# earth-insights/ZoomEarth

Measured on NVIDIA B200. Metric: vision tokens/s crop->patchify->ViT, higher is better.
Workload: dtype fp16

## Files before the change

include/zoomvit.h:

```cpp
#ifndef ZOOMVIT_H_
#define ZOOMVIT_H_

#include <stddef.h>
#include <stdint.h>

#ifdef __cplusplus
extern "C" {
#endif

#define ZV_API __attribute__((visibility("default")))

typedef enum zv_err {
  ZV_OK = 0,
  ZV_EINVAL = -1,
  ZV_EINVAL_ASPECT = -2,
  ZV_EINVAL_BOX = -3,
  ZV_ENOMEM = -4,
  ZV_ECUDA = -5,
  ZV_ENODEV = -6,
  ZV_EARCH = -7
} zv_err;

enum { ZV_F32 = 0, ZV_BF16 = 1, ZV_F16 = 2 };
enum { ZV_ORDER_HF = 0, ZV_ORDER_WINDOW = 1 };
enum { ZV_TOWER_QWEN25 = 0, ZV_TOWER_QWEN2 = 1 };

typedef struct zv_cfg {
  int32_t patch;
  int32_t merge;
  int32_t temporal;
  int32_t window;
  int32_t min_size;
  int32_t depth;
  int32_t hidden;
  int32_t heads;
  int32_t inter;
  int32_t out_hidden;
  int32_t fullatt_mask_lo;
  int32_t op_dtype;
  int64_t min_pixels;
  int64_t max_pixels;
  double  rescale;
  float   mean[3];
  float   std[3];
  float   eps;
  float   reserved_f;
  int32_t tower_kind;
  int32_t reserved_i;
} zv_cfg;

ZV_API const char* zv_version(void);
ZV_API const char* zv_last_error(void);
ZV_API void zv_default_cfg(zv_cfg* cfg);

ZV_API int zv_cut_box(int32_t img_w, int32_t img_h, const double* bbox_xyxy, int32_t min_size, int32_t* box_out4);
ZV_API int zv_resize_dims(int32_t w, int32_t h, int32_t max_size, int32_t* new_wh2, double* inv_scale);
ZV_API int zv_resize_dims_ex(int32_t w, int32_t h, int32_t max_size, int32_t mode, int32_t* new_wh2, double* inv_scale);
ZV_API int zv_cut_box_sft(int32_t img_w, int32_t img_h, const double* bbox_xyxy, int32_t min_size, int32_t* box_out4,
                          int32_t* resized_wh2, int32_t* centre_box4);
ZV_API int zv_smart_resize(int32_t height, int32_t width, int32_t factor, int64_t min_pixels, int64_t max_pixels,
                           int32_t* out_hw2);
ZV_API int zv_geometry(const zv_cfg* cfg, int32_t n, const int32_t* img_hw, const double* bbox_xyxy,
                       int32_t* crop_box, int32_t* resized_hw, int64_t* grid_thw);

ZV_API int32_t zv_resample_ksize(int32_t in_size, int32_t out_size);
ZV_API int zv_resample_coeffs(int32_t in_size, int32_t out_size, int32_t* bounds, int32_t* kk);
ZV_API int zv_normalize_lut(const zv_cfg* cfg, float* lut768);

ZV_API int64_t zv_preprocess_workspace_bytes(int32_t n, const int32_t* crop_box, const int32_t* resized_hw);
ZV_API int zv_preprocess(const zv_cfg* cfg, int32_t n, const uint8_t* const* src_dev, const int32_t* src_hw,
                         const int64_t* src_pitch, const int32_t* crop_box, const int32_t* resized_hw,
                         const int64_t* row_off, void* out_dev, int32_t out_dtype, int32_t row_order,
                         void* workspace_dev, int64_t workspace_bytes, void* stream);

ZV_API int64_t zv_resize_u8_workspace_bytes(int32_t n, const int32_t* crop_box, const int32_t* out_hw);
ZV_API int zv_resize_u8(int32_t n, const uint8_t* const* src_dev, const int32_t* src_hw, const int64_t* src_pitch,
                        const int32_t* crop_box, const int32_t* out_hw, uint8_t* const* dst_dev, const int64_t* dst_pitch,
                        void* workspace_dev, int64_t workspace_bytes, void* stream);

ZV_API int zv_debug_k1_tc_host(const zv_cfg* cfg, int32_t n, const uint8_t* const* src_host, const int32_t* src_hw,
                               const int64_t* src_pitch, const int32_t* crop_box, const int32_t* resized_hw, float* out_host,
                               int32_t row_order, uint8_t* const* u8_dst_host, const int64_t* u8_pitch, void* workspace_host,
                               int64_t workspace_bytes, int32_t* took_tc);

typedef struct zv_plan zv_plan;
ZV_API int zv_plan_create(const zv_cfg* cfg, int32_t n, const int64_t* grid_thw, zv_plan** out);
ZV_API void zv_plan_free(zv_plan* p);
ZV_API int64_t zv_plan_num_patches(const zv_plan* p);
ZV_API int64_t zv_plan_num_tokens(const zv_plan* p);
ZV_API const int64_t* zv_plan_window_index(const zv_plan* p);
ZV_API const int64_t* zv_plan_reverse_index(const zv_plan* p);
ZV_API const int32_t* zv_plan_cu_window(const zv_plan* p, int32_t* n_out);
ZV_API const int32_t* zv_plan_cu_window_raw(const zv_plan* p, int32_t* n_out);
ZV_API const int32_t* zv_plan_cu_full(const zv_plan* p, int32_t* n_out);
ZV_API const int32_t* zv_plan_pos_ids(const zv_plan* p);
ZV_API int64_t zv_plan_device_bytes(const zv_plan* p);
ZV_API int zv_plan_upload(zv_plan* p, void* plan_dev, int64_t bytes, void* stream);

typedef struct zv_tensor {
  const char* name;
  const void* data;
  int32_t dtype;
  int32_t ndim;
  int64_t shape[5];
} zv_tensor;
ZV_API int64_t zv_weights_bytes(const zv_cfg* cfg);
ZV_API int zv_weights_pack(const zv_cfg* cfg, const zv_tensor* tensors, int32_t n, void* packed_dev,
                           int64_t packed_bytes, void* stream);

ZV_API int64_t zv_visual_workspace_bytes(const zv_cfg* cfg, const zv_plan* p);
ZV_API int zv_visual_forward(const zv_cfg* cfg, const void* weights_dev, const zv_plan* p, const void* plan_dev,
                             const void* patches_dev, int32_t in_dtype, int32_t in_order, void* merged_out_dev,
                             int32_t out_dtype, void* hidden_out_dev, void* workspace_dev,
                             int64_t workspace_bytes, void* stream);
ZV_API int zv_visual_forward_gather(const zv_cfg* cfg, const void* weights_dev, const zv_plan* p, const void* plan_dev,
                                    const void* patches_dev, int32_t in_dtype, int32_t in_order, void* merged_out_dev,
                                    int32_t out_dtype, void* workspace_dev, int64_t workspace_bytes,
                                    void* const* peer_out_dev, int32_t n_peers, int64_t peer_row_off, void* stream);
ZV_API int zv_visual_forward_gather_rows(const zv_cfg* cfg, const void* weights_dev, const zv_plan* p, const void* plan_dev,
                                         const void* patches_dev, int32_t in_dtype, int32_t in_order, void* gather_local_dev,
                                         int64_t gather_rows, int32_t out_dtype, const int64_t* dest_rows_dev,
                                         void* workspace_dev, int64_t workspace_bytes, void* const* peer_out_dev,
                                         int32_t n_peers, void* stream);
ZV_API int zv_visual_forward_into(const zv_cfg* cfg, const void* weights_dev, const zv_plan* p, const void* plan_dev,
                                  const void* patches_dev, int32_t in_dtype, int32_t in_order, void* embeds_dev,
                                  int64_t embeds_rows, int32_t embeds_dtype, const int64_t* dest_rows_dev,
                                  void* workspace_dev, int64_t workspace_bytes, void* stream);

ZV_API int zv_rope_index(const int64_t* input_ids, const int64_t* attention_mask, int32_t batch, int32_t seq_len,
                         const int64_t* image_grid_thw, int32_t n_images, int64_t image_token_id,
                         int64_t video_token_id, int64_t vision_start_token_id, int32_t merge, int32_t hf5_semantics,
                         int64_t* position_ids, int64_t* deltas);
ZV_API int64_t zv_placeholder_rows(const int64_t* input_ids, int64_t n_tokens, int64_t image_token_id,
                                   int64_t* rows_out, int64_t rows_cap);

ZV_API int64_t zv_last_launch_count(void);

ZV_API void zv_timing_enable(int on);
ZV_API void zv_timing_reset(void);
ZV_API int zv_timing_read(int kernel_class, double* ms_total, int64_t* count);

ZV_API int zv_gemm_bf16(const void* a_dev, int64_t lda, const void* b_dev, int64_t ldb, const float* bias_dev,
                        void* c_dev, int64_t ldc, int32_t c_dtype, int64_t m, int64_t n, int64_t k,
                        void* stream);
ZV_API int zv_gemm_ex(int32_t epilogue, const void* a_dev, int64_t lda, const void* b_dev, int64_t ldb,
                      const float* bias_dev, void* out_dev, int64_t ldo, int32_t out_dtype, int64_t m, int64_t n,
                      int64_t k, const int32_t* pos_dev, const float* rope_dev, const int32_t* scatter_dev,
                      int32_t heads, int32_t op_dtype , void* stream);
ZV_API int zv_attention(const void* qkv_dev, void* out_dev, int32_t heads, int32_t head_dim,
                        const int32_t* cu_seqlens_host, int32_t n_seg, void* work_dev, int64_t work_bytes,
                        int32_t dtype , void* stream);

#ifdef __cplusplus
}
#endif
#endif
```

zoomearth_b200/_lib.py:

```python
import ctypes as C
import os

_HERE = os.path.dirname(os.path.abspath(__file__))
LIB_PATH = os.path.join(_HERE, "libzoomvit.so")

ZV_F32, ZV_BF16, ZV_F16 = 0, 1, 2
ORDER_HF, ORDER_WINDOW = 0, 1
TOWER_QWEN25, TOWER_QWEN2 = 0, 1
ZV_EINVAL, ZV_EINVAL_ASPECT, ZV_EINVAL_BOX, ZV_ENOMEM, ZV_ECUDA, ZV_ENODEV, ZV_EARCH = -1, -2, -3, -4, -5, -6, -7


class ZvCfg(C.Structure):
    _fields_ = [
        ("patch", C.c_int32), ("merge", C.c_int32), ("temporal", C.c_int32), ("window", C.c_int32),
        ("min_size", C.c_int32), ("depth", C.c_int32), ("hidden", C.c_int32), ("heads", C.c_int32),
        ("inter", C.c_int32), ("out_hidden", C.c_int32), ("fullatt_mask_lo", C.c_int32), ("op_dtype", C.c_int32),
        ("min_pixels", C.c_int64), ("max_pixels", C.c_int64), ("rescale", C.c_double),
        ("mean", C.c_float * 3), ("std", C.c_float * 3), ("eps", C.c_float), ("reserved_f", C.c_float),
        ("tower_kind", C.c_int32), ("reserved_i", C.c_int32),
    ]


class ZvTensor(C.Structure):
    _fields_ = [("name", C.c_char_p), ("data", C.c_void_p), ("dtype", C.c_int32), ("ndim", C.c_int32),
                ("shape", C.c_int64 * 5)]


class ZoomVitError(RuntimeError):
    def __init__(self, code, msg):
        super().__init__(f"libzoomvit error {code}: {msg}")
        self.code = code
        self.msg = msg


_P = C.POINTER
_PROTOS = {
    "zv_version": (C.c_char_p, []),
    "zv_last_error": (C.c_char_p, []),
    "zv_default_cfg": (None, [_P(ZvCfg)]),
    "zv_cut_box": (C.c_int, [C.c_int32, C.c_int32, _P(C.c_double), C.c_int32, _P(C.c_int32)]),
    "zv_resize_dims": (C.c_int, [C.c_int32, C.c_int32, C.c_int32, _P(C.c_int32), _P(C.c_double)]),
    "zv_resize_dims_ex": (C.c_int, [C.c_int32, C.c_int32, C.c_int32, C.c_int32, _P(C.c_int32), _P(C.c_double)]),
    "zv_cut_box_sft": (C.c_int, [C.c_int32, C.c_int32, _P(C.c_double), C.c_int32, _P(C.c_int32), _P(C.c_int32), _P(C.c_int32)]),
    "zv_resize_u8_workspace_bytes": (C.c_int64, [C.c_int32, C.c_void_p, C.c_void_p]),
    "zv_resize_u8": (C.c_int, [C.c_int32, C.c_void_p, C.c_void_p, C.c_void_p, C.c_void_p, C.c_void_p, C.c_void_p, C.c_void_p,
                              C.c_void_p, C.c_int64, C.c_void_p]),
    "zv_smart_resize": (C.c_int, [C.c_int32, C.c_int32, C.c_int32, C.c_int64, C.c_int64, _P(C.c_int32)]),
    "zv_geometry": (C.c_int, [_P(ZvCfg), C.c_int32, C.c_void_p, C.c_void_p, C.c_void_p, C.c_void_p, C.c_void_p]),
    "zv_resample_ksize": (C.c_int32, [C.c_int32, C.c_int32]),
    "zv_resample_coeffs": (C.c_int, [C.c_int32, C.c_int32, C.c_void_p, C.c_void_p]),
    "zv_normalize_lut": (C.c_int, [_P(ZvCfg), C.c_void_p]),
    "zv_preprocess_workspace_bytes": (C.c_int64, [C.c_int32, C.c_void_p, C.c_void_p]),
    "zv_preprocess": (C.c_int, [_P(ZvCfg), C.c_int32, C.c_void_p, C.c_void_p, C.c_void_p, C.c_void_p, C.c_void_p,
                                C.c_void_p, C.c_void_p, C.c_int32, C.c_int32, C.c_void_p, C.c_int64, C.c_void_p]),
    "zv_debug_k1_tc_host": (C.c_int, [_P(ZvCfg), C.c_int32, C.c_void_p, C.c_void_p, C.c_void_p, C.c_void_p, C.c_void_p, C.c_void_p,
                                     C.c_int32, C.c_void_p, C.c_void_p, C.c_void_p, C.c_int64, C.c_void_p]),
    "zv_plan_create": (C.c_int, [_P(ZvCfg), C.c_int32, C.c_void_p, _P(C.c_void_p)]),
    "zv_plan_free": (None, [C.c_void_p]),
    "zv_plan_num_patches": (C.c_int64, [C.c_void_p]),
    "zv_plan_num_tokens": (C.c_int64, [C.c_void_p]),
    "zv_plan_window_index": (_P(C.c_int64), [C.c_void_p]),
    "zv_plan_reverse_index": (_P(C.c_int64), [C.c_void_p]),
    "zv_plan_cu_window": (_P(C.c_int32), [C.c_void_p, _P(C.c_int32)]),
    "zv_plan_cu_window_raw": (_P(C.c_int32), [C.c_void_p, _P(C.c_int32)]),
    "zv_plan_cu_full": (_P(C.c_int32), [C.c_void_p, _P(C.c_int32)]),
    "zv_plan_pos_ids": (_P(C.c_int32), [C.c_void_p]),
    "zv_plan_device_bytes": (C.c_int64, [C.c_void_p]),
    "zv_plan_upload": (C.c_int, [C.c_void_p, C.c_void_p, C.c_int64, C.c_void_p]),
    "zv_weights_bytes": (C.c_int64, [_P(ZvCfg)]),
    "zv_weights_pack": (C.c_int, [_P(ZvCfg), _P(ZvTensor), C.c_int32, C.c_void_p, C.c_int64, C.c_void_p]),
    "zv_visual_workspace_bytes": (C.c_int64, [_P(ZvCfg), C.c_void_p]),
    "zv_visual_forward": (C.c_int, [_P(ZvCfg), C.c_void_p, C.c_void_p, C.c_void_p, C.c_void_p, C.c_int32, C.c_int32,
                                    C.c_void_p, C.c_int32, C.c_void_p, C.c_void_p, C.c_int64, C.c_void_p]),
    "zv_visual_forward_gather": (C.c_int, [_P(ZvCfg), C.c_void_p, C.c_void_p, C.c_void_p, C.c_void_p, C.c_int32, C.c_int32,
                                           C.c_void_p, C.c_int32, C.c_void_p, C.c_int64, C.c_void_p, C.c_int32, C.c_int64,
                                           C.c_void_p]),
    "zv_visual_forward_gather_rows": (C.c_int, [_P(ZvCfg), C.c_void_p, C.c_void_p, C.c_void_p, C.c_void_p, C.c_int32, C.c_int32,
                                                C.c_void_p, C.c_int64, C.c_int32, C.c_void_p, C.c_void_p, C.c_int64, C.c_void_p,
                                                C.c_int32, C.c_void_p]),
    "zv_visual_forward_into": (C.c_int, [_P(ZvCfg), C.c_void_p, C.c_void_p, C.c_void_p, C.c_void_p, C.c_int32, C.c_int32,
                                         C.c_void_p, C.c_int64, C.c_int32, C.c_void_p, C.c_void_p, C.c_int64, C.c_void_p]),
    "zv_rope_index": (C.c_int, [C.c_void_p, C.c_void_p, C.c_int32, C.c_int32, C.c_void_p, C.c_int32, C.c_int64, C.c_int64,
                                C.c_int64, C.c_int32, C.c_int32, C.c_void_p, C.c_void_p]),
    "zv_placeholder_rows": (C.c_int64, [C.c_void_p, C.c_int64, C.c_int64, C.c_void_p, C.c_int64]),
    "zv_last_launch_count": (C.c_int64, []),
    "zv_timing_enable": (None, [C.c_int]),
    "zv_timing_reset": (None, []),
    "zv_timing_read": (C.c_int, [C.c_int, _P(C.c_double), _P(C.c_int64)]),
    "zv_gemm_bf16": (C.c_int, [C.c_void_p, C.c_int64, C.c_void_p, C.c_int64, C.c_void_p, C.c_void_p, C.c_int64,
                               C.c_int32, C.c_int64, C.c_int64, C.c_int64, C.c_void_p]),
    "zv_gemm_ex": (C.c_int, [C.c_int32, C.c_void_p, C.c_int64, C.c_void_p, C.c_int64, C.c_void_p, C.c_void_p, C.c_int64,
                             C.c_int32, C.c_int64, C.c_int64, C.c_int64, C.c_void_p, C.c_void_p, C.c_void_p, C.c_int32,
                             C.c_int32, C.c_void_p]),
    "zv_attention": (C.c_int, [C.c_void_p, C.c_void_p, C.c_int32, C.c_int32, C.c_void_p, C.c_int32, C.c_void_p,
                               C.c_int64, C.c_int32, C.c_void_p]),
}
EXPORTS = tuple(_PROTOS)
_lib = None


def lib():
    global _lib
    if _lib is None:
        if not os.path.exists(LIB_PATH):
            raise ImportError(
                f"{LIB_PATH} is missing: run `python -m zoomearth_b200.build` (nvcc, sm_100a). "
                "zoomearth_b200 has no CPU or PyTorch fallback path.")
        handle = C.CDLL(LIB_PATH)
        for name, (res, args) in _PROTOS.items():
            fn = getattr(handle, name)
            fn.restype = res
            fn.argtypes = args
        _lib = handle
    return _lib


def check(rc):
    if rc is not None and rc < 0:
        raise ZoomVitError(rc, lib().zv_last_error().decode())
    return rc


def default_cfg(**overrides):
    cfg = ZvCfg()
    lib().zv_default_cfg(C.byref(cfg))
    for k, v in overrides.items():
        if k in ("mean", "std"):
            setattr(cfg, k, (C.c_float * 3)(*v))
        elif k == "fullatt":
            m = 0
            for i in v:
                m |= 1 << i
            cfg.fullatt_mask_lo = m - (1 << 32) if m >= (1 << 31) else m
        else:
            setattr(cfg, k, v)
    return cfg
```

zoomearth_b200/csrc/zv_gemm.cu:

```cuda
#include <cuda.h>
#include <cuda_bf16.h>
#include <cuda_fp16.h>
#include <cuda_runtime.h>

#include <cstdlib>
#include <mutex>

#include "zv_common.h"
#include "zv_gemm.h"
#include "zv_ptx.cuh"

namespace zv {

using namespace ptx;

namespace {

constexpr int BM = 128, BK = 64, UMMA_K = 16;
constexpr int kThreads = 384;
constexpr int kTmemCols = 512;

constexpr int kXposePitch = 36;
constexpr int kXposeBytesPerWarp = 32 * kXposePitch * 4;
constexpr int kQkvRope0 = 24 * 32 * 8, kQkvRope1 = 16 * 32 * 8, kQkvTilePitch = 88, kQkvTile = 32 * kQkvTilePitch * 2;
constexpr int kQkvStageBytes = 4 * kQkvRope0 + 4 * kQkvRope1 + 4 * kQkvTile;
__host__ __device__ constexpr bool is_resid(int e) { return e == EPI_RESID || e == EPI_RESID_LN; }
__host__ __device__ constexpr bool is_qkv(int e) { return e == EPI_QKV_ROPE || e == EPI_QKV_ROPE_LN; }
template <int BN, int CG, int EPI = 0> struct Cfg {
  static constexpr int kBRows = BN / CG;
  static constexpr int kABytes = BM * BK * 2;
  static constexpr int kBBytes = kBRows * BK * 2;
  static constexpr int kStageBytes = kABytes + kBBytes;
  static constexpr int kXposeBytes = (is_resid(EPI) || EPI == EPI_SCATTER) ? 8 * kXposeBytesPerWarp : is_qkv(EPI) ? kQkvStageBytes : 0;
  static constexpr int kStages = ((kBRows > 128) ? 4 : 6) - ((is_resid(EPI) || is_qkv(EPI) || EPI == EPI_SCATTER) ? 1 : 0);
  static constexpr int kBarBytes = 256;
  static constexpr int kSmemBytes = kStages * kStageBytes + kBarBytes + kXposeBytes + 1024;
};

__device__ __forceinline__ float silu(float x) { return __fdividef(x, 1.0f + __expf(-x)); }
__device__ __forceinline__ float quick_gelu(float x) { return __fdividef(x, 1.0f + __expf(-1.702f * x)); }
__device__ __forceinline__ float gelu_erf(float x) { return 0.5f * x * (1.0f + erff(x * 0.70710678118654752440f)); }
__device__ __forceinline__ uint32_t pack2(float a, float b, bool f16) {
  if (f16) { __half2 v = __floats2half2_rn(a, b); return *reinterpret_cast<uint32_t*>(&v); }
  __nv_bfloat162 v = __floats2bfloat162_rn(a, b);
  return *reinterpret_cast<uint32_t*>(&v);
}
__device__ __forceinline__ void tmem_ld_x8(uint32_t taddr, uint32_t (&r)[8]) {
  asm volatile("tcgen05.ld.sync.aligned.32x32b.x8.b32 {%0, %1, %2, %3, %4, %5, %6, %7}, [%8];"
               : "=r"(r[0]), "=r"(r[1]), "=r"(r[2]), "=r"(r[3]), "=r"(r[4]), "=r"(r[5]), "=r"(r[6]), "=r"(r[7])
               : "r"(taddr) : "memory");
}
__device__ __forceinline__ void load_bias32(const float* __restrict__ b, float (&v)[32]) {
  const float4* p = reinterpret_cast<const float4*>(b);
#pragma unroll
  for (int j = 0; j < 8; ++j) { const float4 t = __ldg(p + j); v[4 * j] = t.x; v[4 * j + 1] = t.y; v[4 * j + 2] = t.z; v[4 * j + 3] = t.w; }
}

__device__ __forceinline__ float row_rscale(const GemmArgs& g, int row, bool valid) {
  if (g.row_ss == nullptr || !valid) return 1.f;
  const float2* p = reinterpret_cast<const float2*>(g.row_ss + (int64_t)row * kSsParts);
  float s = 0.f;
#pragma unroll
  for (int i = 0; i < kSsParts / 2; ++i) { const float2 t = __ldg(p + i); s += t.x; s += t.y; }
  return rsqrtf(s / (float)g.norm_dim + g.norm_eps);
}

__device__ __forceinline__ void row_ln_stats(const GemmArgs& g, int row, bool valid, float& mu, float& rs) {
  mu = 0.f; rs = 1.f;
  if (!valid) return;
  const float4* p = reinterpret_cast<const float4*>(g.row_ln + (int64_t)row * kSsParts);
  float mean = 0.f, m2 = 0.f;
#pragma unroll
  for (int i = 0; i < kSsParts / 2; ++i) {
    const float4 t = __ldg(p + i);
#pragma unroll
    for (int h = 0; h < 2; ++h) {
      const int k = 2 * i + h;
      const float mb = h ? t.z : t.x, m2b = h ? t.w : t.y;
      if (k == 0) { mean = mb; m2 = m2b; continue; }
      const float d = mb - mean;
      mean = fmaf(d, 1.f / (float)(k + 1), mean);
      m2 += fmaf(d * d, 64.f * (float)k / (float)(k + 1), m2b);
    }
  }
  mu = mean;
  rs = rsqrtf(m2 / (float)g.norm_dim + g.norm_eps);
}

template <int BN, int EPI, typename WaitFn>
__device__ __forceinline__ void epilogue_tile(uint32_t taddr, int m_blk, int n_blk, int row_local, int half,
                                              const GemmArgs& g, float* xpose, WaitFn wait_accumulator) {
  const int row = m_blk * BM + row_local;
  const bool valid = row < g.M;
  const bool of16 = g.out_dtype == ZV_F16;
  if constexpr (!is_resid(EPI) && EPI != EPI_QKV_ROPE_LN && EPI != EPI_QGELU) wait_accumulator();
  if constexpr (is_resid(EPI)) {
    constexpr int HALF = BN / 2;
    const int lane = row_local & 31;
    const int rr = lane >> 3, cc = (lane & 7) * 4;
    const int row_base = m_blk * BM + (row_local & ~31);
    float* xrow = static_cast<float*>(g.out) + (int64_t)row_base * g.ldo + n_blk * BN + half * HALF + cc;
    float4 xv[8];
    auto load_x = [&](int c) {
#pragma unroll
      for (int i = 0; i < 8; ++i) {
        const int r = 4 * i + rr;
        xv[i] = (row_base + r < g.M) ? *reinterpret_cast<const float4*>(xrow + (int64_t)r * g.ldo + c) : make_float4(0.f, 0.f, 0.f, 0.f);
      }
    };
    const bool emit = g.x16_out != nullptr;
    uint16_t* x16row = static_cast<uint16_t*>(g.x16_out) + (int64_t)row_base * g.N + n_blk * BN + half * HALF + cc;
    float ssp[8];
#pragma unroll
    for (int i = 0; i < 8; ++i) ssp[i] = 0.f;
    constexpr bool LN = EPI == EPI_RESID_LN;
    float x0[8], s1[8], s2[8];
#pragma unroll
    for (int i = 0; i < 8; ++i) x0[i] = s1[i] = s2[i] = 0.f;
    load_x(0);
    wait_accumulator();
#pragma unroll 1
    for (int c = 0; c < HALF; c += 32) {
      uint32_t r[32];
      __syncwarp();
      tmem_ld_x32(taddr + half * HALF + c, r);
      float v[32];
      load_bias32(g.bias + n_blk * BN + half * HALF + c, v);
      tmem_ld_wait();
#pragma unroll
      for (int j = 0; j < 8; ++j)
        *reinterpret_cast<float4*>(xpose + lane * kXposePitch + 4 * j) =
            make_float4(v[4 * j] + __uint_as_float(r[4 * j]), v[4 * j + 1] + __uint_as_float(r[4 * j + 1]),
                        v[4 * j + 2] + __uint_as_float(r[4 * j + 2]), v[4 * j + 3] + __uint_as_float(r[4 * j + 3]));
      __syncwarp();
#pragma unroll
      for (int i = 0; i < 8; ++i) {
        const int rw = 4 * i + rr;
        const float4 a = *reinterpret_cast<const float4*>(xpose + rw * kXposePitch + cc);
        if (row_base + rw < g.M) {
          const float4 nx = make_float4(xv[i].x + a.x, xv[i].y + a.y, xv[i].z + a.z, xv[i].w + a.w);
          *reinterpret_cast<float4*>(xrow + (int64_t)rw * g.ldo + c) = nx;
          if (emit) {
            *reinterpret_cast<uint2*>(x16row + (int64_t)rw * g.N + c) = make_uint2(pack2(nx.x, nx.y, g.op_f16 != 0), pack2(nx.z, nx.w, g.op_f16 != 0));
            if constexpr (!LN) ssp[i] += nx.x * nx.x + nx.y * nx.y + nx.z * nx.z + nx.w * nx.w;
          }
        }
        if constexpr (LN) {
          if (emit) {
            const float4 nx = make_float4(xv[i].x + a.x, xv[i].y + a.y, xv[i].z + a.z, xv[i].w + a.w);
            if (c == 0) x0[i] = __shfl_sync(0xffffffffu, nx.x, lane & ~7);
            const float dx = nx.x - x0[i], dy = nx.y - x0[i], dz = nx.z - x0[i], dw = nx.w - x0[i];
            s1[i] += (dx + dy) + (dz + dw);
            s2[i] += (dx * dx + dy * dy) + (dz * dz + dw * dw);
          }
        }
      }
      if (c + 32 < HALF) load_x(c + 32);
    }
    if (LN && emit) {
#pragma unroll
      for (int i = 0; i < 8; ++i) {
        float a1 = s1[i], a2 = s2[i];
#pragma unroll
        for (int o = 1; o < 8; o <<= 1) { a1 += __shfl_xor_sync(0xffffffffu, a1, o); a2 += __shfl_xor_sync(0xffffffffu, a2, o); }
        const float mean_off = a1 / (float)HALF;
        const float m2 = fmaxf(fmaf(-a1, mean_off, a2), 0.f);
        const int rw = 4 * i + rr;
        if ((lane & 7) == 0 && row_base + rw < g.M) {
          float2* o = g.ln_out + (int64_t)(row_base + rw) * kSsParts + (n_blk * BN + half * HALF) / 64;
          if (HALF == 128) { o[0] = o[1] = make_float2(x0[i] + mean_off, 0.5f * m2); }
          else o[0] = make_float2(x0[i] + mean_off, m2);
        }
      }
    } else if (emit) {
#pragma unroll
      for (int i = 0; i < 8; ++i) {
        float v = ssp[i];
        v += __shfl_xor_sync(0xffffffffu, v, 1);
        v += __shfl_xor_sync(0xffffffffu, v, 2);
        v += __shfl_xor_sync(0xffffffffu, v, 4);
        const int rw = 4 * i + rr;
        if ((lane & 7) == 0 && row_base + rw < g.M)
          g.ss_out[(int64_t)(row_base + rw) * kSsParts + (n_blk * BN + half * HALF) / 64] = v;
      }
    }
  } else if constexpr (EPI == EPI_STORE || EPI == EPI_GELU || EPI == EPI_SCATTER || EPI == EPI_QGELU) {
    constexpr int HALF = BN / 2;
    int64_t orow = row;
    bool keep = valid;
    float mu = 0.f, rs = 1.f;
    if constexpr (EPI == EPI_QGELU) {
      row_ln_stats(g, row, valid, mu, rs);
      wait_accumulator();
    }
    if constexpr (EPI == EPI_SCATTER) { orow = valid ? (int64_t)__ldg(g.scatter + row) : 0; keep = valid && orow >= 0; }
    const int c_begin = half * HALF;
#pragma unroll 1
    for (int c = c_begin; c < c_begin + HALF; c += 32) {
      uint32_t r[32];
      __syncwarp();
      tmem_ld_x32(taddr + c, r);
      const int n0 = n_blk * BN + c;
      float v[32];
      if (g.bias) load_bias32(g.bias + n0, v);
      else {
#pragma unroll
        for (int j = 0; j < 32; ++j) v[j] = 0.f;
      }
      if constexpr (EPI == EPI_QGELU) {
        float cs[32];
        load_bias32(g.colsum + n0, cs);
        tmem_ld_wait();
#pragma unroll
        for (int j = 0; j < 32; ++j) v[j] = quick_gelu(fmaf(fmaf(-mu, cs[j], __uint_as_float(r[j])), rs, v[j]));
      } else {
        tmem_ld_wait();
#pragma unroll
        for (int j = 0; j < 32; ++j) v[j] += __uint_as_float(r[j]);
      }
      if constexpr (EPI == EPI_GELU) {
#pragma unroll
        for (int j = 0; j < 32; ++j) v[j] = gelu_erf(v[j]);
      }
      if (keep) {
        if (g.out_dtype == ZV_F32) {
          float4* o = reinterpret_cast<float4*>(static_cast<float*>(g.out) + orow * g.ldo + n0);
#pragma unroll
          for (int j = 0; j < 8; ++j) o[j] = make_float4(v[4 * j], v[4 * j + 1], v[4 * j + 2], v[4 * j + 3]);
        } else {
          uint4 pk[4];
#pragma unroll
          for (int j = 0; j < 4; ++j)
            pk[j] = make_uint4(pack2(v[8 * j], v[8 * j + 1], of16), pack2(v[8 * j + 2], v[8 * j + 3], of16),
                               pack2(v[8 * j + 4], v[8 * j + 5], of16), pack2(v[8 * j + 6], v[8 * j + 7], of16));
          if constexpr (EPI != EPI_SCATTER) {
            uint4* o = reinterpret_cast<uint4*>(static_cast<__nv_bfloat16*>(g.out) + orow * g.ldo + n0);
#pragma unroll
            for (int j = 0; j < 4; ++j) o[j] = pk[j];
          } else {
            uint4* st = reinterpret_cast<uint4*>(reinterpret_cast<uint8_t*>(xpose) + (row_local & 31) * 80);
#pragma unroll
            for (int j = 0; j < 4; ++j) st[j] = pk[j];
          }
        }
      }
      if constexpr (EPI == EPI_SCATTER) {
        if (g.out_dtype != ZV_F32) {
          __syncwarp();
          const int ln = row_local & 31, piece = ln & 3;
          const int row_base = m_blk * BM + (row_local & ~31);
#pragma unroll
          for (int i = 0; i < 4; ++i) {
            const int rw = 8 * i + (ln >> 2);
            const int64_t dr = row_base + rw < g.M ? (int64_t)__ldg(g.scatter + row_base + rw) : -1;
            if (dr >= 0) {
              const uint4 val = *reinterpret_cast<const uint4*>(reinterpret_cast<const uint8_t*>(xpose) + rw * 80 + piece * 16);
              *reinterpret_cast<uint4*>(static_cast<__nv_bfloat16*>(g.out) + dr * g.ldo + n0 + piece * 8) = val;
              for (int p = 0; p < g.n_peers; ++p)
                *reinterpret_cast<uint4*>(static_cast<__nv_bfloat16*>(g.peers[p]) + (g.peer_row_off + dr) * g.ldo + n0 + piece * 8) = val;
            }
          }
          __syncwarp();
        }
      }
    }
  } else if constexpr (EPI == EPI_SWIGLU) {
    static_assert(EPI != EPI_SWIGLU || BN == 256, "SwiGLU tiles hold 128 gate + 128 up columns");
    const float rs = row_rscale(g, row, valid);
#pragma unroll 1
    for (int c = half * 64; c < half * 64 + 64; c += 32) {
      uint32_t a[32], b[32];
      __syncwarp();
      tmem_ld_x32(taddr + c, a);
      tmem_ld_x32(taddr + 128 + c, b);
      float bg[32], bu[32];
      load_bias32(g.bias + (int64_t)n_blk * 256 + c, bg);
      load_bias32(g.bias + (int64_t)n_blk * 256 + 128 + c, bu);
      tmem_ld_wait();
      uint32_t o[16];
#pragma unroll
      for (int j = 0; j < 16; ++j) {
        const float g0 = fmaf(__uint_as_float(a[2 * j]), rs, bg[2 * j]), g1 = fmaf(__uint_as_float(a[2 * j + 1]), rs, bg[2 * j + 1]);
        const float u0 = fmaf(__uint_as_float(b[2 * j]), rs, bu[2 * j]), u1 = fmaf(__uint_as_float(b[2 * j + 1]), rs, bu[2 * j + 1]);
        o[j] = pack2(silu(g0) * u0, silu(g1) * u1, of16);
      }
      if (valid) {
        uint4* dst = reinterpret_cast<uint4*>(static_cast<__nv_bfloat16*>(g.out) + (int64_t)row * g.ldo + n_blk * 128 + c);
#pragma unroll
        for (int j = 0; j < 4; ++j) dst[j] = make_uint4(o[4 * j], o[4 * j + 1], o[4 * j + 2], o[4 * j + 3]);
      }
    }
  } else if constexpr (is_qkv(EPI)) {
    static_assert(!is_qkv(EPI) || BN == 240, "QKV tiles hold three 80-wide heads");
    const int lane = row_local & 31, q = row_local >> 5;
    uint8_t* stage = reinterpret_cast<uint8_t*>(xpose);
    float2* ropeS = reinterpret_cast<float2*>(stage + (half == 0 ? q * kQkvRope0 : 4 * kQkvRope0 + q * kQkvRope1));
    uint16_t* tileS = reinterpret_cast<uint16_t*>(stage + 4 * kQkvRope0 + 4 * kQkvRope1 + q * kQkvTile);
    const int NP = half == 0 ? 24 : 16, P0 = half == 0 ? 0 : 24;
    {
      int ph = 0, pw = 0;
      if (valid) { ph = __ldg(g.pos + 2 * row); pw = __ldg(g.pos + 2 * row + 1); }
      const float2* rope_h = g.rope + (int64_t)ph * 20;
      const float2* rope_w = g.rope + (int64_t)pw * 20;
      for (int d = 0; d < NP; ++d) {
        const int pair = P0 + d;
        ropeS[d * 32 + lane] = pair < 20 ? __ldg(rope_h + pair) : __ldg(rope_w + (pair - 20));
      }
    }
    float mu = 0.f, rs;
    if constexpr (EPI == EPI_QKV_ROPE_LN) row_ln_stats(g, row, valid, mu, rs);
// ... 80 lines not shown
  }
}

__device__ __forceinline__ uint32_t cluster_ctarank() {
  uint32_t r;
  asm volatile("mov.u32 %0, %%cluster_ctarank;" : "=r"(r));
  return r;
}
__device__ __forceinline__ void cluster_sync_all() {
  asm volatile("barrier.cluster.arrive.release.aligned;" ::: "memory");
  asm volatile("barrier.cluster.wait.acquire.aligned;" ::: "memory");
}
__device__ __forceinline__ void tma_load_2d_pair(void* smem_dst, const void* tmap, uint64_t* bar, int32_t c0, int32_t c1) {
  asm volatile(
      "cp.async.bulk.tensor.2d.cta_group::2.shared::cluster.global.mbarrier::complete_tx::bytes [%0], [%1, {%3, %4}], [%2];"
      ::"r"(smem_u32(smem_dst)), "l"(tmap), "r"(smem_u32(bar) & 0xFEFFFFFFu), "r"(c0), "r"(c1)
      : "memory");
}
__device__ __forceinline__ void umma_pair(uint32_t tmem_d, uint64_t desc_a, uint64_t desc_b, uint32_t idesc, uint32_t accumulate) {
  asm volatile(
      "{\n\t.reg .pred p;\n\tsetp.ne.b32 p, %4, 0;\n\ttcgen05.mma.cta_group::2.kind::f16 [%0], %1, %2, %3, p;\n\t}"
      ::"r"(tmem_d), "l"(desc_a), "l"(desc_b), "r"(idesc), "r"(accumulate)
      : "memory");
}
__device__ __forceinline__ void umma_commit_pair(uint64_t* bar) {
  asm volatile("tcgen05.commit.cta_group::2.mbarrier::arrive::one.shared::cluster.multicast::cluster.b64 [%0], %1;"
               ::"r"(smem_u32(bar)), "h"((uint16_t)3) : "memory");
}
__device__ __forceinline__ void mbar_arrive_cta(uint64_t* bar, uint32_t cta) {
  asm volatile(
      "{\n\t.reg .b32 ra;\n\tmapa.shared::cluster.u32 ra, %0, %1;\n\tmbarrier.arrive.shared::cluster.b64 _, [ra];\n\t}"
      ::"r"(smem_u32(bar)), "r"(cta) : "memory");
}
__device__ __forceinline__ void tmem_alloc_pair(uint32_t* smem_slot, uint32_t ncols) {
  asm volatile("tcgen05.alloc.cta_group::2.sync.aligned.shared::cta.b32 [%0], %1;" ::"r"(smem_u32(smem_slot)), "r"(ncols) : "memory");
  asm volatile("tcgen05.relinquish_alloc_permit.cta_group::2.sync.aligned;" ::: "memory");
}
__device__ __forceinline__ void tmem_dealloc_pair(uint32_t taddr, uint32_t ncols) {
  asm volatile("tcgen05.dealloc.cta_group::2.sync.aligned.b32 %0, %1;" ::"r"(taddr), "r"(ncols) : "memory");
}

template <int BN, int EPI, int CG>
__global__ void __launch_bounds__(kThreads, 1) gemm_tc(const __grid_constant__ CUtensorMap tma_a,
                                                       const __grid_constant__ CUtensorMap tma_b, const GemmArgs g) {
  using C = Cfg<BN, CG, EPI>;
  extern __shared__ uint8_t smem_raw[];
  uint8_t* smem = reinterpret_cast<uint8_t*>((reinterpret_cast<uintptr_t>(smem_raw) + 1023) & ~(uintptr_t)1023);
  uint64_t* bars = reinterpret_cast<uint64_t*>(smem + C::kStages * C::kStageBytes);
  uint64_t* full = bars;
  uint64_t* empty = bars + C::kStages;
  uint64_t* tfull = bars + 2 * C::kStages;
  uint64_t* tempty = tfull + 2;
  uint32_t* tmem_slot = reinterpret_cast<uint32_t*>(tempty + 2);

  const int warp = threadIdx.x >> 5, lane = threadIdx.x & 31;
  const uint32_t rank = CG == 2 ? cluster_ctarank() : 0;
  const bool leader = rank == 0;
  const int n_blocks = g.N / BN;
  const int m_blocks = (g.M + BM * CG - 1) / (BM * CG);
  const int num_tiles = m_blocks * n_blocks;
  const int k_blocks = (g.K + BK - 1) / BK;
  const int first_tile = blockIdx.x / CG, tile_step = gridDim.x / CG;

  if (threadIdx.x == 0) {
    prefetch_tensormap(&tma_a);
    prefetch_tensormap(&tma_b);
    for (int s = 0; s < C::kStages; ++s) { mbar_init(full + s, 1); mbar_init(empty + s, 1); }
    for (int a = 0; a < 2; ++a) { mbar_init(tfull + a, 1); mbar_init(tempty + a, 8 * CG); }
    fence_mbar_init();
  }
  if (warp == 2) {
    if constexpr (CG == 2) tmem_alloc_pair(tmem_slot, kTmemCols);
    else { tmem_alloc(tmem_slot, kTmemCols); tmem_relinquish(); }
  }
  tc_fence_before();
  if constexpr (CG == 2) cluster_sync_all(); else __syncthreads();
  tc_fence_after();
  const uint32_t tmem_base = *tmem_slot;
  if (warp != 0) pdl_wait();

  if (warp == 0) {
    if (elect_one()) {
      int stage = 0; uint32_t phase = 0;
      bool first_pass = first_tile < num_tiles;
      if (first_pass) {
        const int n_row = (first_tile % n_blocks) * BN + (int)rank * C::kBRows;
        const int pre = k_blocks < C::kStages ? k_blocks : C::kStages;
        for (int kb = 0; kb < pre; ++kb) {
          uint8_t* sa = smem + kb * C::kStageBytes;
          if constexpr (CG == 2) {
            if (leader) mbar_arrive_expect_tx(full + kb, 2 * C::kStageBytes);
            tma_load_2d_pair(sa + C::kABytes, &tma_b, full + kb, kb * BK, n_row);
          } else {
            mbar_arrive_expect_tx(full + kb, C::kStageBytes);
            tma_load_2d(sa + C::kABytes, &tma_b, full + kb, kb * BK, n_row);
          }
        }
      }
      pdl_wait();
      for (int tile = first_tile; tile < num_tiles; tile += tile_step) {
        const int m_row = (tile / n_blocks) * BM * CG + (int)rank * BM;
        const int n_row = (tile % n_blocks) * BN + (int)rank * C::kBRows;
        for (int kb = 0; kb < k_blocks; ++kb) {
          uint8_t* sa = smem + stage * C::kStageBytes;
          const bool b_requested = first_pass && kb < C::kStages;
          if (!b_requested) mbar_wait(empty + stage, phase ^ 1);
          if constexpr (CG == 2) {
            if (!b_requested && leader) mbar_arrive_expect_tx(full + stage, 2 * C::kStageBytes);
            tma_load_2d_pair(sa, &tma_a, full + stage, kb * BK, m_row);
            if (!b_requested) tma_load_2d_pair(sa + C::kABytes, &tma_b, full + stage, kb * BK, n_row);
          } else {
            if (!b_requested) mbar_arrive_expect_tx(full + stage, C::kStageBytes);
            tma_load_2d(sa, &tma_a, full + stage, kb * BK, m_row);
            if (!b_requested) tma_load_2d(sa + C::kABytes, &tma_b, full + stage, kb * BK, n_row);
          }
          if (++stage == C::kStages) { stage = 0; phase ^= 1; }
        }
        first_pass = false;
      }
      pdl_trigger();
    }
  } else if (warp == 1) {
    if (leader && elect_one()) {
      const uint32_t idesc = umma_idesc_16bit(BM * CG, BN, g.op_f16 != 0);
      int stage = 0; uint32_t phase = 0;
      int it = 0;
      for (int tile = first_tile; tile < num_tiles; tile += tile_step, ++it) {
        const int acc = it & 1;
        const uint32_t acc_phase = (it >> 1) & 1;
        mbar_wait(tempty + acc, acc_phase ^ 1);
        tc_fence_after();
        const uint32_t tmem_d = tmem_base + acc * 256;
        for (int kb = 0; kb < k_blocks; ++kb) {
          mbar_wait(full + stage, phase);
          tc_fence_after();
          const uint32_t sa = smem_u32(smem + stage * C::kStageBytes);
          const uint64_t da = umma_desc_k128(sa), db = umma_desc_k128(sa + C::kABytes);
#pragma unroll
          for (int k = 0; k < BK / UMMA_K; ++k) {
            if constexpr (CG == 2) umma_pair(tmem_d, da + 2 * k, db + 2 * k, idesc, (kb | k) != 0);
            else umma_bf16(tmem_d, da + 2 * k, db + 2 * k, idesc, (kb | k) != 0);
          }
          if constexpr (CG == 2) umma_commit_pair(empty + stage); else umma_commit(empty + stage);
          if (++stage == C::kStages) { stage = 0; phase ^= 1; }
        }
        if constexpr (CG == 2) umma_commit_pair(tfull + acc); else umma_commit(tfull + acc);
      }
    }
  } else if (warp >= 4) {
    const int q = warp & 3, half = (warp - 4) >> 2;
    float* xpose = reinterpret_cast<float*>(smem + C::kStages * C::kStageBytes + C::kBarBytes) +
                   ((is_resid(EPI) || EPI == EPI_SCATTER) ? (warp - 4) * (kXposeBytesPerWarp / 4) : 0);
    int it = 0;
    for (int tile = first_tile; tile < num_tiles; tile += tile_step, ++it) {
      const int m_blk = (tile / n_blocks) * CG + (int)rank, n_blk = tile % n_blocks;
      const int acc = it & 1;
      const uint32_t acc_phase = (it >> 1) & 1;
      const uint32_t taddr = tmem_base + acc * 256 + ((uint32_t)(q * 32) << 16);
      epilogue_tile<BN, EPI>(taddr, m_blk, n_blk, q * 32 + lane, half, g, xpose, [&] {
        mbar_wait(tfull + acc, acc_phase);
        tc_fence_after();
      });
      tc_fence_before();
      __syncwarp();
      if (lane == 0) {
        if constexpr (CG == 2) mbar_arrive_cta(tempty + acc, 0); else mbar_arrive(tempty + acc);
      }
    }
  }
  tc_fence_before();
  if constexpr (CG == 2) cluster_sync_all(); else __syncthreads();
  if (warp == 2) {
    tc_fence_after();
    if constexpr (CG == 2) tmem_dealloc_pair(tmem_base, kTmemCols); else tmem_dealloc(tmem_base, kTmemCols);
  }
}

typedef CUresult (*EncodeTiledFn)(CUtensorMap*, CUtensorMapDataType, cuuint32_t, void*, const cuuint64_t*,
                                  const cuuint64_t*, const cuuint32_t*, const cuuint32_t*, CUtensorMapInterleave,
                                  CUtensorMapSwizzle, CUtensorMapL2promotion, CUtensorMapFloatOOBfill);

}
int make_tmap_2d(void* tm, const void* base, int64_t rows, int64_t cols, int64_t ld, int box_cols, int box_rows,
                 int swizzle_bytes, bool f16);
namespace {

EncodeTiledFn encode_fn() {
  static EncodeTiledFn fn = nullptr;
  static std::once_flag once;
  std::call_once(once, [] {
    void* p = nullptr;
    cudaDriverEntryPointQueryResult q;
    if (cudaGetDriverEntryPoint("cuTensorMapEncodeTiled", &p, cudaEnableDefault, &q) == cudaSuccess &&
        q == cudaDriverEntryPointSuccess)
      fn = reinterpret_cast<EncodeTiledFn>(p);
  });
  return fn;
}

int make_tmap(CUtensorMap* tm, const void* base, int64_t rows, int64_t cols, int64_t ld, int box_rows, bool f16) {
  return make_tmap_2d(tm, base, rows, cols, ld, BK, box_rows, 128, f16);
}

template <int BN, int EPI, int CG>
int launch(const GemmArgs& g, const void* a, int64_t lda, const void* b, int64_t ldb, cudaStream_t stream) {
  using C = Cfg<BN, CG, EPI>;
  if (g.N % BN) return fail(ZV_EINVAL, "gemm: N=%d is not a multiple of the %d-wide tile", g.N, BN);
  CUtensorMap ta, tb;
  int rc = make_tmap(&ta, a, g.M, g.K, lda, BM, g.op_f16 != 0);
  if (rc) return rc;
  rc = make_tmap(&tb, b, g.N, g.K, ldb, C::kBRows, g.op_f16 != 0);
  if (rc) return rc;
  static std::atomic<uint64_t> attr_set{0};
  const int dev = current_device();
  if (device_needs_setup(attr_set, dev)) {
    cudaError_t e = cudaFuncSetAttribute(gemm_tc<BN, EPI, CG>, cudaFuncAttributeMaxDynamicSharedMemorySize, C::kSmemBytes);
    if (e != cudaSuccess) return fail(ZV_ECUDA, "gemm: cudaFuncSetAttribute: %s", cudaGetErrorString(e));
    mark_device(attr_set, dev);
  }
  const int tiles = ((g.M + BM * CG - 1) / (BM * CG)) * (g.N / BN);
  const int slots = num_sms() / CG;
  const int grid = (tiles < slots ? tiles : slots) * CG;
  cudaError_t e;
  {
    static const char* const kNames[] = {"zv:K2 gemm store", "zv:K2 gemm qkv+rope", "zv:K2 gemm residual", "zv:K2 gemm swiglu",
                                         "zv:K2 gemm gelu", "zv:K2 gemm scatter", "zv:K2 gemm qkv+ln+rope",
                                         "zv:K2 gemm residual+ln", "zv:K2 gemm quickgelu"};
    NvtxRange nvtx(kNames[EPI]);
    KernelTimer timer(is_qkv(EPI) ? KC_GEMM_QKV : is_resid(EPI) ? KC_GEMM_RESID : EPI == EPI_QGELU ? KC_GEMM_QGELU : KC_GEMM_STORE + EPI, stream);
    e = launch_pdl(gemm_tc<BN, EPI, CG>, dim3((unsigned)grid), dim3(kThreads), C::kSmemBytes, stream, CG, ta, tb, g);
  }
  count_launch();
  if (e == cudaSuccess) e = cudaGetLastError();
  if (e != cudaSuccess) return fail(ZV_ECUDA, "gemm: launch: %s", cudaGetErrorString(e));
  return ZV_OK;
}

}

int make_tmap_2d(void* tm_, const void* base, int64_t rows, int64_t cols, int64_t ld, int box_cols, int box_rows,
                 int swizzle_bytes, bool f16) {
  CUtensorMap* tm = static_cast<CUtensorMap*>(tm_);
  EncodeTiledFn fn = encode_fn();
  if (!fn) return fail(ZV_ECUDA, "tma: cuTensorMapEncodeTiled is not available from the driver");
  if ((reinterpret_cast<uintptr_t>(base) & 15) || (ld * 2) % 16)
    return fail(ZV_EINVAL, "tma: operand base/pitch must be 16-byte aligned (base %p, ld %lld)", base, (long long)ld);
  cuuint64_t dims[2] = {(cuuint64_t)cols, (cuuint64_t)rows};
  cuuint64_t strides[1] = {(cuuint64_t)ld * 2};
  cuuint32_t box[2] = {(cuuint32_t)box_cols, (cuuint32_t)box_rows};
  cuuint32_t estr[2] = {1, 1};
  const CUtensorMapSwizzle sw = swizzle_bytes == 128 ? CU_TENSOR_MAP_SWIZZLE_128B
                                : swizzle_bytes == 64 ? CU_TENSOR_MAP_SWIZZLE_64B
                                : swizzle_bytes == 32 ? CU_TENSOR_MAP_SWIZZLE_32B : CU_TENSOR_MAP_SWIZZLE_NONE;
  CUresult r = fn(tm, f16 ? CU_TENSOR_MAP_DATA_TYPE_FLOAT16 : CU_TENSOR_MAP_DATA_TYPE_BFLOAT16, 2, const_cast<void*>(base),
                  dims, strides, box, estr, CU_TENSOR_MAP_INTERLEAVE_NONE, sw, CU_TENSOR_MAP_L2_PROMOTION_L2_256B,
                  CU_TENSOR_MAP_FLOAT_OOB_FILL_NONE);
  if (r != CUDA_SUCCESS) return fail(ZV_ECUDA, "tma: cuTensorMapEncodeTiled failed with CUresult %d", (int)r);
  return ZV_OK;
}

int make_tmap_u8(void* tm_, const void* base, uint64_t dim0, uint64_t dim1, uint64_t stride1, int box0, int box1) {
  CUtensorMap* tm = static_cast<CUtensorMap*>(tm_);
  EncodeTiledFn fn = encode_fn();
  if (!fn) return fail(ZV_ECUDA, "tma: cuTensorMapEncodeTiled is not available from the driver");
  if ((reinterpret_cast<uintptr_t>(base) & 15) || stride1 % 16 || dim0 == 0 || dim1 == 0)
    return fail(ZV_EINVAL, "tma: uint8 operand base/pitch must be 16-byte aligned (base %p, pitch %llu)", base, (unsigned long long)stride1);
  cuuint64_t dims[2] = {(cuuint64_t)dim0, (cuuint64_t)dim1};
  cuuint64_t strides[1] = {(cuuint64_t)stride1};
  cuuint32_t box[2] = {(cuuint32_t)box0, (cuuint32_t)box1};
  cuuint32_t estr[2] = {1, 1};
  CUresult r = fn(tm, CU_TENSOR_MAP_DATA_TYPE_UINT8, 2, const_cast<void*>(base), dims, strides, box, estr,
                  CU_TENSOR_MAP_INTERLEAVE_NONE, CU_TENSOR_MAP_SWIZZLE_128B, CU_TENSOR_MAP_L2_PROMOTION_L2_256B,
                  CU_TENSOR_MAP_FLOAT_OOB_FILL_NONE);
  if (r != CUDA_SUCCESS) return fail(ZV_ECUDA, "tma: cuTensorMapEncodeTiled (uint8) failed with CUresult %d", (int)r);
  return ZV_OK;
}

int gemm(int epi, const GemmArgs& g, const void* a, int64_t lda, const void* b, int64_t ldb, void* stream_) {
  cudaStream_t stream = static_cast<cudaStream_t>(stream_);
  if (g.M <= 0 || g.N <= 0 || g.K <= 0) return fail(ZV_EINVAL, "gemm: empty problem %dx%dx%d", g.M, g.N, g.K);
#ifdef ZV_DEBUG_GEMM_1CTA
  {
    switch (epi) {
      case EPI_STORE:
        return g.N % 256 == 0 ? launch<256, EPI_STORE, 1>(g, a, lda, b, ldb, stream)
                              : launch<128, EPI_STORE, 1>(g, a, lda, b, ldb, stream);
      case EPI_QKV_ROPE: return launch<240, EPI_QKV_ROPE, 1>(g, a, lda, b, ldb, stream);
      case EPI_RESID: return launch<256, EPI_RESID, 1>(g, a, lda, b, ldb, stream);
      case EPI_SWIGLU: return launch<256, EPI_SWIGLU, 1>(g, a, lda, b, ldb, stream);
      case EPI_GELU: return launch<256, EPI_GELU, 1>(g, a, lda, b, ldb, stream);
      case EPI_SCATTER: return launch<256, EPI_SCATTER, 1>(g, a, lda, b, ldb, stream);
      case EPI_QKV_ROPE_LN: return launch<240, EPI_QKV_ROPE_LN, 1>(g, a, lda, b, ldb, stream);
      case EPI_RESID_LN: return launch<256, EPI_RESID_LN, 1>(g, a, lda, b, ldb, stream);
      case EPI_QGELU: return launch<256, EPI_QGELU, 1>(g, a, lda, b, ldb, stream);
    }
  }
#endif
  switch (epi) {
    case EPI_STORE:
      return g.N % 256 == 0 ? launch<256, EPI_STORE, 2>(g, a, lda, b, ldb, stream)
                            : launch<128, EPI_STORE, 1>(g, a, lda, b, ldb, stream);
    case EPI_QKV_ROPE: return launch<240, EPI_QKV_ROPE, 2>(g, a, lda, b, ldb, stream);
    case EPI_RESID:
    case EPI_RESID_LN: {
      const int64_t slots = num_sms() / 2, mp = (g.M + 2 * BM - 1) / (2 * BM);
      const int64_t cost256 = 2 * ((mp * (g.N / 256) + slots - 1) / slots), cost128 = (mp * (g.N / 128) + slots - 1) / slots;
      const bool wide = g.N % 256 == 0 && 5 * cost128 > 4 * cost256;
      if (epi == EPI_RESID_LN)
        return wide ? launch<256, EPI_RESID_LN, 2>(g, a, lda, b, ldb, stream) : launch<128, EPI_RESID_LN, 2>(g, a, lda, b, ldb, stream);
      if (wide) return launch<256, EPI_RESID, 2>(g, a, lda, b, ldb, stream);
      return launch<128, EPI_RESID, 2>(g, a, lda, b, ldb, stream);
    }
    case EPI_SWIGLU: return launch<256, EPI_SWIGLU, 2>(g, a, lda, b, ldb, stream);
    case EPI_GELU: return launch<256, EPI_GELU, 2>(g, a, lda, b, ldb, stream);
    case EPI_SCATTER: return launch<256, EPI_SCATTER, 2>(g, a, lda, b, ldb, stream);
    case EPI_QKV_ROPE_LN: return launch<240, EPI_QKV_ROPE_LN, 2>(g, a, lda, b, ldb, stream);
    case EPI_QGELU: return launch<256, EPI_QGELU, 2>(g, a, lda, b, ldb, stream);
  }
  return fail(ZV_EINVAL, "gemm: unknown epilogue %d", epi);
}

}

extern "C" int zv_gemm_bf16(const void* a_dev, int64_t lda, const void* b_dev, int64_t ldb, const float* bias_dev,
                            void* c_dev, int64_t ldc, int32_t c_dtype, int64_t m, int64_t n, int64_t k, void* stream) {
  zv::reset_launch_count();
  if (!a_dev || !b_dev || !c_dev) return zv::fail(ZV_EINVAL, "zv_gemm_bf16: null pointer");
  if (n % 128) return zv::fail(ZV_EINVAL, "zv_gemm_bf16: N must be a multiple of 128");
  if (c_dtype != ZV_F32 && c_dtype != ZV_BF16) return zv::fail(ZV_EINVAL, "zv_gemm_bf16: bad c_dtype");
  zv::GemmArgs g{};
  g.M = (int)m; g.N = (int)n; g.K = (int)k;
  g.out = c_dev; g.ldo = ldc; g.out_dtype = c_dtype; g.bias = bias_dev;
  return zv::gemm(zv::EPI_STORE, g, a_dev, lda, b_dev, ldb, stream);
}

extern "C" int zv_gemm_ex(int32_t epilogue, const void* a_dev, int64_t lda, const void* b_dev, int64_t ldb,
                          const float* bias_dev, void* out_dev, int64_t ldo, int32_t out_dtype, int64_t m, int64_t n,
                          int64_t k, const int32_t* pos_dev, const float* rope_dev, const int32_t* scatter_dev,
                          int32_t heads, int32_t op_dtype, void* stream) {
  zv::reset_launch_count();
  if (!a_dev || !b_dev || !out_dev) return zv::fail(ZV_EINVAL, "zv_gemm_ex: null pointer");
  if (epilogue < zv::EPI_STORE || epilogue > zv::EPI_SCATTER) return zv::fail(ZV_EINVAL, "gemm: unknown epilogue %d", epilogue);
  zv::GemmArgs g{};
  g.M = (int)m; g.N = (int)n; g.K = (int)k;
  g.out = out_dev; g.ldo = ldo; g.out_dtype = out_dtype; g.bias = bias_dev;
  g.pos = pos_dev; g.rope = reinterpret_cast<const float2*>(rope_dev); g.scatter = scatter_dev; g.heads = heads;
  g.op_f16 = op_dtype == ZV_F16;
  if (epilogue != zv::EPI_STORE && !bias_dev) return zv::fail(ZV_EINVAL, "zv_gemm_ex: this epilogue needs a bias");
  if (epilogue == zv::EPI_QKV_ROPE && (!pos_dev || !rope_dev)) return zv::fail(ZV_EINVAL, "zv_gemm_ex: rope tables missing");
  if (epilogue == zv::EPI_SCATTER && !scatter_dev) return zv::fail(ZV_EINVAL, "zv_gemm_ex: scatter index missing");
  return zv::gemm(epilogue, g, a_dev, lda, b_dev, ldb, stream);
}
```

Measured before the change: 183,100.

## Prefetch residual rows across chunks and tiles in the residual GEMM epilogue

The residual epilogue now loads the next 32-column chunk of the fp32 residual stream while the current chunk is processed. On the last chunk it loads the first chunk of the next tile this CTA owns and carries it in registers across tiles, so global-load latency overlaps the TMEM load and the wait for the accumulator. The bias add moves after the transpose, using one float4 per lane instead of 32 scalar bias loads per lane. A debug entry point for the residual GEMM is also added. The extra prefetch buffer raises register pressure in the epilogue warps.

```diff
diff --git a/include/zoomvit.h b/include/zoomvit.h
--- a/include/zoomvit.h
+++ b/include/zoomvit.h
@@ -147,6 +147,9 @@
                       const float* bias_dev, void* out_dev, int64_t ldo, int32_t out_dtype, int64_t m, int64_t n,
                       int64_t k, const int32_t* pos_dev, const float* rope_dev, const int32_t* scatter_dev,
                       int32_t heads, int32_t op_dtype , void* stream);
+ZV_API int zv_debug_gemm_resid(int32_t epilogue, const void* a_dev, int64_t lda, const void* b_dev, int64_t ldb,
+                               const float* bias_dev, float* x_dev, int64_t ldx, int64_t m, int64_t n, int64_t k,
+                               void* x16_dev, void* stats_dev, int32_t op_dtype, void* stream);
 ZV_API int zv_attention(const void* qkv_dev, void* out_dev, int32_t heads, int32_t head_dim,
                         const int32_t* cu_seqlens_host, int32_t n_seg, void* work_dev, int64_t work_bytes,
                         int32_t dtype , void* stream);
diff --git a/zoomearth_b200/_lib.py b/zoomearth_b200/_lib.py
--- a/zoomearth_b200/_lib.py
+++ b/zoomearth_b200/_lib.py
@@ -92,6 +92,9 @@
     "zv_gemm_ex": (C.c_int, [C.c_int32, C.c_void_p, C.c_int64, C.c_void_p, C.c_int64, C.c_void_p, C.c_void_p, C.c_int64,
                              C.c_int32, C.c_int64, C.c_int64, C.c_int64, C.c_void_p, C.c_void_p, C.c_void_p, C.c_int32,
                              C.c_int32, C.c_void_p]),
+    "zv_debug_gemm_resid": (C.c_int, [C.c_int32, C.c_void_p, C.c_int64, C.c_void_p, C.c_int64, C.c_void_p, C.c_void_p,
+                                      C.c_int64, C.c_int64, C.c_int64, C.c_int64, C.c_void_p, C.c_void_p, C.c_int32,
+                                      C.c_void_p]),
     "zv_attention": (C.c_int, [C.c_void_p, C.c_void_p, C.c_int32, C.c_int32, C.c_void_p, C.c_int32, C.c_void_p,
                                C.c_int64, C.c_int32, C.c_void_p]),
 }
diff --git a/zoomearth_b200/csrc/zv_gemm.cu b/zoomearth_b200/csrc/zv_gemm.cu
--- a/zoomearth_b200/csrc/zv_gemm.cu
+++ b/zoomearth_b200/csrc/zv_gemm.cu
@@ -89,7 +89,8 @@
 
 template <int BN, int EPI, typename WaitFn>
 __device__ __forceinline__ void epilogue_tile(uint32_t taddr, int m_blk, int n_blk, int row_local, int half,
-                                              const GemmArgs& g, float* xpose, WaitFn wait_accumulator) {
+                                              const GemmArgs& g, float* xpose, WaitFn wait_accumulator,
+                                              float4 (&xv)[8], bool carried, int next_m_blk, int next_n_blk) {
   const int row = m_blk * BM + row_local;
   const bool valid = row < g.M;
   const bool of16 = g.out_dtype == ZV_F16;
@@ -99,13 +100,17 @@
     const int lane = row_local & 31;
     const int rr = lane >> 3, cc = (lane & 7) * 4;
     const int row_base = m_blk * BM + (row_local & ~31);
-    float* xrow = static_cast<float*>(g.out) + (int64_t)row_base * g.ldo + n_blk * BN + half * HALF + cc;
-    float4 xv[8];
-    auto load_x = [&](int c) {
+    auto x_at = [&](int mb, int nb) {
+      return static_cast<float*>(g.out) + (int64_t)(mb * BM + (row_local & ~31)) * g.ldo + nb * BN + half * HALF + cc;
+    };
+    float* xrow = x_at(m_blk, n_blk);
+    const float* brow = g.bias + n_blk * BN + half * HALF + cc;
+    float4 xn[8];
+    auto load_x = [&](int rb, const float* src, float4 (&dst)[8]) {
 #pragma unroll
       for (int i = 0; i < 8; ++i) {
         const int r = 4 * i + rr;
-        xv[i] = (row_base + r < g.M) ? *reinterpret_cast<const float4*>(xrow + (int64_t)r * g.ldo + c) : make_float4(0.f, 0.f, 0.f, 0.f);
+        dst[i] = (rb + r < g.M) ? *reinterpret_cast<const float4*>(src + (int64_t)r * g.ldo) : make_float4(0.f, 0.f, 0.f, 0.f);
       }
     };
     const bool emit = g.x16_out != nullptr;
@@ -117,26 +122,26 @@
     float x0[8], s1[8], s2[8];
 #pragma unroll
     for (int i = 0; i < 8; ++i) x0[i] = s1[i] = s2[i] = 0.f;
-    load_x(0);
+    if (!carried) load_x(row_base, xrow, xv);
     wait_accumulator();
 #pragma unroll 1
     for (int c = 0; c < HALF; c += 32) {
       uint32_t r[32];
       __syncwarp();
       tmem_ld_x32(taddr + half * HALF + c, r);
-      float v[32];
-      load_bias32(g.bias + n_blk * BN + half * HALF + c, v);
+      if (c + 32 < HALF) load_x(row_base, xrow + c + 32, xn);
+      else if (next_m_blk >= 0) load_x(next_m_blk * BM + (row_local & ~31), x_at(next_m_blk, next_n_blk), xn);
       tmem_ld_wait();
 #pragma unroll
       for (int j = 0; j < 8; ++j)
-        *reinterpret_cast<float4*>(xpose + lane * kXposePitch + 4 * j) =
-            make_float4(v[4 * j] + __uint_as_float(r[4 * j]), v[4 * j + 1] + __uint_as_float(r[4 * j + 1]),
-                        v[4 * j + 2] + __uint_as_float(r[4 * j + 2]), v[4 * j + 3] + __uint_as_float(r[4 * j + 3]));
+        *reinterpret_cast<uint4*>(xpose + lane * kXposePitch + 4 * j) = make_uint4(r[4 * j], r[4 * j + 1], r[4 * j + 2], r[4 * j + 3]);
+      const float4 b = __ldg(reinterpret_cast<const float4*>(brow + c));
       __syncwarp();
 #pragma unroll
       for (int i = 0; i < 8; ++i) {
         const int rw = 4 * i + rr;
-        const float4 a = *reinterpret_cast<const float4*>(xpose + rw * kXposePitch + cc);
+        const float4 t = *reinterpret_cast<const float4*>(xpose + rw * kXposePitch + cc);
+        const float4 a = make_float4(b.x + t.x, b.y + t.y, b.z + t.z, b.w + t.w);
         if (row_base + rw < g.M) {
           const float4 nx = make_float4(xv[i].x + a.x, xv[i].y + a.y, xv[i].z + a.z, xv[i].w + a.w);
           *reinterpret_cast<float4*>(xrow + (int64_t)rw * g.ldo + c) = nx;
@@ -155,7 +160,8 @@
           }
         }
       }
-      if (c + 32 < HALF) load_x(c + 32);
+#pragma unroll
+      for (int i = 0; i < 8; ++i) xv[i] = xn[i];
     }
     if (LN && emit) {
 #pragma unroll
@@ -542,15 +548,17 @@
     float* xpose = reinterpret_cast<float*>(smem + C::kStages * C::kStageBytes + C::kBarBytes) +
                    ((is_resid(EPI) || EPI == EPI_SCATTER) ? (warp - 4) * (kXposeBytesPerWarp / 4) : 0);
     int it = 0;
+    float4 xcarry[8];
     for (int tile = first_tile; tile < num_tiles; tile += tile_step, ++it) {
       const int m_blk = (tile / n_blocks) * CG + (int)rank, n_blk = tile % n_blocks;
       const int acc = it & 1;
       const uint32_t acc_phase = (it >> 1) & 1;
       const uint32_t taddr = tmem_base + acc * 256 + ((uint32_t)(q * 32) << 16);
+      const int next = tile + tile_step;
       epilogue_tile<BN, EPI>(taddr, m_blk, n_blk, q * 32 + lane, half, g, xpose, [&] {
         mbar_wait(tfull + acc, acc_phase);
         tc_fence_after();
-      });
+      }, xcarry, it > 0, next < num_tiles ? (next / n_blocks) * CG + (int)rank : -1, next % n_blocks);
       tc_fence_before();
       __syncwarp();
       if (lane == 0) {
@@ -741,3 +749,22 @@
   if (epilogue == zv::EPI_SCATTER && !scatter_dev) return zv::fail(ZV_EINVAL, "zv_gemm_ex: scatter index missing");
   return zv::gemm(epilogue, g, a_dev, lda, b_dev, ldb, stream);
 }
+
+extern "C" int zv_debug_gemm_resid(int32_t epilogue, const void* a_dev, int64_t lda, const void* b_dev, int64_t ldb,
+                                   const float* bias_dev, float* x_dev, int64_t ldx, int64_t m, int64_t n, int64_t k,
+                                   void* x16_dev, void* stats_dev, int32_t op_dtype, void* stream) {
+  zv::reset_launch_count();
+  if (!a_dev || !b_dev || !bias_dev || !x_dev) return zv::fail(ZV_EINVAL, "zv_debug_gemm_resid: null pointer");
+  if (epilogue != zv::EPI_RESID && epilogue != zv::EPI_RESID_LN)
+    return zv::fail(ZV_EINVAL, "zv_debug_gemm_resid: epilogue %d is not a residual epilogue", epilogue);
+  if (n % 128 || n > 64 * zv::kSsParts) return zv::fail(ZV_EINVAL, "zv_debug_gemm_resid: N=%lld is not a multiple of 128 <= %d", (long long)n, 64 * zv::kSsParts);
+  if (!x16_dev != !stats_dev) return zv::fail(ZV_EINVAL, "zv_debug_gemm_resid: x16 and row statistics go together");
+  zv::GemmArgs g{};
+  g.M = (int)m; g.N = (int)n; g.K = (int)k;
+  g.out = x_dev; g.ldo = ldx; g.out_dtype = ZV_F32; g.bias = bias_dev;
+  g.op_f16 = op_dtype == ZV_F16;
+  g.x16_out = x16_dev;
+  if (epilogue == zv::EPI_RESID) g.ss_out = static_cast<float*>(stats_dev);
+  else g.ln_out = static_cast<float2*>(stats_dev);
+  return zv::gemm(epilogue, g, a_dev, lda, b_dev, ldb, stream);
+}
```

New measurement: 183,400, median of 6. Within noise of the previous version (+0.2%).
